# bmds-lab/Crackling

Hardware: AMD Instinct MI355X
Metric: guides/sec (whole node) + achieved HBM GB/s, 20bp/<=4mm ISSL scan (higher is better)
Workload: dtype u32

## Files before the change

crackling_amd/csrc/issl_bin.hip:

```cpp
#include <hip/hip_runtime.h>

#include <algorithm>
#include <type_traits>

#include "issl_kernels.hpp"

namespace issl {


__global__ __launch_bounds__(256) void k_pack_scan_stream(ImageView v, uint32_t *__restrict__ scan_out,
                                                          uint64_t *__restrict__ esig_out,
                                                          uint8_t *__restrict__ occ8_out,
                                                          uint32_t *__restrict__ error_flag, uint32_t *__restrict__ seen,
                                                          uint32_t tile_begin, uint32_t tile_end)
{
    for (uint32_t t = tile_begin + blockIdx.x; t < tile_end; t += gridDim.x) {
        uint32_t lo = 0, hi = v.n_buckets;
        while (hi - lo > 1) {
            const uint32_t mid = (lo + hi) >> 1;
            if (v.tile_first[mid] <= t) lo = mid; else hi = mid;
        }
        const uint32_t b = lo;
        const uint32_t slice = b >> v.slice_width;
        const uint64_t start = v.bucket_start[b];
// ... 463 lines not shown
                                                   ScanItem *__restrict__ fitems, uint32_t item_guides, uint32_t tail_shapes,
                                                   FineItemLds<THREADS> &l)
{
    const uint32_t w = threadIdx.x;
    const FineSum base = fbase[b];
    const uint64_t blen = v.bucket_start[b + 1] - v.bucket_start[b];
    const uint32_t tile_first_b = v.tile_first[b];
    uint32_t c = 0, c1 = 0, s0 = 0, s1 = 0;
    if (w < 256u) {
        c = fcount[static_cast<uint64_t>(b) * 256u + w];
        c1 = c - fcount0[static_cast<uint64_t>(b) * 256u + w];
        const uint32_t *ss = v.sub_start + static_cast<uint64_t>(b) * 257u;
        s0 = ss[w];
        s1 = ss[w + 1];
    }
    uint64_t cost = 0, slots = 0, items = 0;
    GroupUnits gu{};
    if (c) {
        gu = group_units(s0, s1, tail_shapes);
        const uint32_t kk = (c + item_guides - 1u) / item_guides;
        slots = (c + kGuideGroup - 1u) / kGuideGroup * kGuideGroup;
        items = static_cast<uint64_t>(gu.units) * kk;
        for (uint32_t done = 0; done < c; done += item_guides) cost += group_cost(gu, c - done < item_guides ? c - done : item_guides);
    }
    const uint64_t cost_at = base.cost + block_exclusive_scan(cost, l.scan, nullptr);
    const uint32_t slot_at = base.slots + static_cast<uint32_t>(block_exclusive_scan(slots, l.scan, nullptr));
    const uint32_t item_at = static_cast<uint32_t>(block_exclusive_scan(items, l.scan, nullptr));
    if (w < 256u) {
        l.item0_of[w] = item_at;
        if (w == 255u) l.item0_of[256] = item_at + static_cast<uint32_t>(items);
        FineGroup g;
        g.cost0 = cost_at; g.chunk_cost = group_cost(gu, item_guides);
        g.s0 = s0; g.s1 = s1; g.n_full = gu.n_full; g.units = gu.units;
        g.shape = gu.shape; g.c = c; g.slot = slot_at; g.slot0 = slot_at + c1;
        l.group[w] = g;
    }
    __syncthreads();
    const uint32_t total = l.item0_of[256];
    for (uint32_t i0 = 0; i0 < total; i0 += THREADS) {
        const uint32_t i = i0 + w;
        if (i < total) {
            uint32_t lo = 0, hi = 256;
            while (hi - lo > 1u) {
                const uint32_t mid = (lo + hi) >> 1;
                if (l.item0_of[mid] <= i) lo = mid; else hi = mid;
            }
            const uint32_t gw = lo;
            const FineGroup g = l.group[gw];
            const uint32_t s0a = g.s0 & ~31u;
            const uint32_t j = i - l.item0_of[gw];
            const uint32_t chunk = j / g.units, t = j - chunk * g.units;
            const uint32_t done = chunk * item_guides;
            const uint32_t len = (g.c - done < item_guides) ? g.c - done : item_guides;
            const bool full = t < g.n_full;
            const uint32_t shape = full ? 32u : g.shape, cap = 64u * shape;
            const uint32_t wstart = s0a + t * kTileCands;
            const uint64_t after = blen - wstart;
            ScanItem it;
            it.bucket = (b << 8) | gw;
            it.g0 = g.slot + done;
            it.g1 = it.g0 + len;
            it.n_tiles = 1;
            it.cost0 = g.cost0 + static_cast<uint64_t>(chunk) * g.chunk_cost +
                       static_cast<uint64_t>(t) * (static_cast<uint64_t>(len) * kGuideCost + kTileFixedCost);
            it.tile0 = base.items + i;
            it.last_cands = after < cap ? static_cast<uint32_t>(after) : cap;
            it.group_abs = tile_first_b * 64u + (wstart >> 5);
            it.window = (t == 0 ? g.s0 - s0a : 0u) | ((g.s1 - wstart < cap ? g.s1 - wstart : cap) << 16);
            it.shape = shape; it.gmid = g.slot0;
            l.stage[w] = it;
        }
        __syncthreads();
        const uint32_t n_here = total - i0 < THREADS ? total - i0 : THREADS;
        const uint4 *src4 = reinterpret_cast<const uint4 *>(l.stage);
        uint4 *dst4 = reinterpret_cast<uint4 *>(fitems + base.items + i0);
        for (uint32_t q = w; q < n_here * 3u; q += THREADS) dst4[q] = src4[q];
        __syncthreads();
    }
}

template <uint32_t WAYS, uint32_t THREADS>
__device__ __forceinline__ void fine_scatter_guides(const ImageView &v, uint32_t b, const uint32_t *__restrict__ gstart,
                                                    const uint32_t *__restrict__ gfill, const uint32_t *__restrict__ gword,
                                                    const uint32_t *__restrict__ gidx, const uint64_t *__restrict__ gsig,
                                                    const uint32_t *__restrict__ fcount, const uint32_t *__restrict__ fcount0,
                                                    const FineSum *__restrict__ fbase, uint32_t *__restrict__ fword,
                                                    FineMeta *__restrict__ fmeta, FineGuideLds<THREADS> &l)
{
    constexpr uint32_t ways = WAYS;
    const uint32_t w = threadIdx.x, slice = b >> v.slice_width;
    const uint32_t g0 = gstart[b], n = gfill[b];
    const uint32_t base_slots = fbase[b].slots;
    uint32_t c = 0, c1 = 0;
    if (w < 256u) {
        c = fcount[static_cast<uint64_t>(b) * 256u + w];
        c1 = c - fcount0[static_cast<uint64_t>(b) * 256u + w];
    }
    uint32_t i = w, guide = 0, word = 0;
    uint64_t sig = 0;
    if (i < n) { guide = gidx[g0 + i]; word = gword[g0 + i]; sig = gsig[g0 + i]; }
    const uint32_t slots = (c + kGuideGroup - 1u) / kGuideGroup * kGuideGroup;
    const uint32_t slot_at = base_slots + static_cast<uint32_t>(block_exclusive_scan(slots, l.scan, nullptr));
    if (w < 256u) {
        l.slot_of[w] = slot_at;
        l.slot0_of[w] = slot_at + c1;
        l.cursor[w] = 0;
        l.cursor0[w] = 0;
        l.has_cands[w] = c ? 1u : 0u;
        for (uint32_t k2 = c; k2 < slots; ++k2) { fmeta[slot_at + k2] = FineMeta{kNoGuide, 0u, 0ull}; fword[slot_at + k2] = kPadGuideWord; }
    }
    __syncthreads();
    while (i < n) {
        const uint32_t gj = succ_byte(sig, slice, v.slice_width);
        const uint32_t word12 = fine_word(word, slice, v.slice_width);
#pragma unroll
        for (uint32_t way = 0; way < ways; ++way) {
            const uint32_t ww = fine_way(gj, way);
            if (!l.has_cands[ww]) continue;
            const uint32_t slot = way ? l.slot_of[ww] + atomicAdd(&l.cursor[ww], 1u) : l.slot0_of[ww] + atomicAdd(&l.cursor0[ww], 1u);
            fword[slot] = word12 | (fine_class(way) << 24);
            fmeta[slot] = FineMeta{guide, (b << 8) | ww, sig};
        }
        i += THREADS;
        if (i < n) { guide = gidx[g0 + i]; word = gword[g0 + i]; sig = gsig[g0 + i]; }
    }
}

template <uint32_t WAYS, uint32_t THREADS>
__global__ __launch_bounds__(THREADS) void k_fine_scatter(ImageView v, const uint32_t *__restrict__ gstart,
                                                          const uint32_t *__restrict__ gfill, const uint32_t *__restrict__ gword,
                                                          const uint32_t *__restrict__ gidx, const uint64_t *__restrict__ gsig,
                                                          const uint32_t *__restrict__ fcount, const uint32_t *__restrict__ fcount0,
                                                          const FineSum *__restrict__ fbase, const PlanInfo *__restrict__ plan,
                                                          uint32_t *__restrict__ fword, FineMeta *__restrict__ fmeta,
                                                          ScanItem *__restrict__ fitems, uint32_t item_guides, uint32_t tail_shapes)
{
    short_kernel_priority();
    if (!plan->fine) return;
    __shared__ union { FineItemLds<THREADS> items; FineGuideLds<THREADS> guides; } lds;
    const uint32_t nb = v.n_buckets;
    if (blockIdx.x < nb) fine_scatter_items(v, blockIdx.x, fcount, fcount0, fbase, fitems, item_guides, tail_shapes, lds.items);
    else fine_scatter_guides<WAYS, THREADS>(v, blockIdx.x - nb, gstart, gfill, gword, gidx, gsig, fcount, fcount0, fbase, fword, fmeta, lds.guides);
}

__global__ __launch_bounds__(256) void k_fine_ranges(const PlanInfo *__restrict__ plan, const ScanItem *__restrict__ fitems,
                                                     RangeStart *__restrict__ starts)
{
    short_kernel_priority();
    if (!plan->fine) return;
    const uint32_t n_ranges = plan->n_ranges;
    const uint32_t r = blockIdx.x * 4u + (threadIdx.x >> 6);
    if (r <= n_ranges && n_ranges != 0) {
        const RangeStart st = range_start_of<true>(fitems, plan->n_items, plan->total_cost, n_ranges, r);
        if ((threadIdx.x & 63u) == 0u) starts[r] = st;
    }
}

constexpr uint32_t kSmallPairs = 512;

__device__ inline uint64_t block512_exclusive_scan(uint64_t v, uint64_t *lds , uint64_t *total)
{
    const uint32_t lane = threadIdx.x & 63u, wave = threadIdx.x >> 6;
    const uint64_t incl = wave_inclusive_scan_u64(v);
    if (lane == 63) lds[wave] = incl;
    __syncthreads();
    uint64_t before = 0, all = 0;
    for (uint32_t w = 0; w < kSmallPairs / 64u; ++w) {
        const uint64_t x = lds[w];
        if (w < wave) before += x;
        all += x;
    }
    if (total) *total = all;
    __syncthreads();
    return before + incl - v;
}

template <uint32_t WAYS>
__global__ __launch_bounds__(kSmallPairs) void k_bin_small(ImageView v, Workspace ws, const uint64_t *__restrict__ guides, uint32_t n,
                                                           uint32_t prune_mode, uint32_t tail_shapes, uint32_t scan_blocks,
                                                           uint32_t sorted_layout)
{
    short_kernel_priority();
    __shared__ uint64_t lds[kSmallPairs / 64u];
    const uint32_t t = threadIdx.x, my_way = blockIdx.x;
    for (uint32_t k = my_way * kSmallPairs + t; k <= n; k += WAYS * kSmallPairs) ws.gcount[k] = 0;
    for (uint32_t k = my_way * kSmallPairs + t; k <= ws.cap_chunks; k += WAYS * kSmallPairs) ws.raw_used[k] = 0;
    if (t == 0 && my_way == 0) {
        ws.scan_span[2u * ws.span_slot] = ~0ull;
        ws.scan_span[2u * ws.span_slot + 1u] = 0ull;
    }
    const uint32_t pairs = n * v.n_slices;
    const uint32_t low = (1u << v.slice_width) - 1u;
    const bool mine = t < pairs;
    const uint32_t g = mine ? t / v.n_slices : 0u, sl = mine ? t - g * v.n_slices : 0u;
    uint64_t sig = 0, blen = 0, units = 0, cost = 0, cand = 0, ref = 0, valid = 0;
    uint64_t cost_before = 0;
    uint32_t units_before = 0, valid_before = 0;
    uint32_t b = 0, gj = 0, tf = 0, my_s0 = 0, my_s1 = 0;
    if (mine) {
        sig = guides[g];
        b = (sl << v.slice_width) + (static_cast<uint32_t>(sig >> (v.slice_width * sl)) & low);
        gj = succ_byte(sig, sl, v.slice_width);
        const uint32_t *ss = v.sub_start + static_cast<uint64_t>(b) * 257u;
        uint32_t s0[WAYS], s1[WAYS];
#pragma unroll
        for (uint32_t way = 0; way < WAYS; ++way) {
            const uint32_t ww = fine_way(gj, way);
            s0[way] = ss[ww];
            s1[way] = ss[ww + 1];
        }
        blen = v.bucket_start[b + 1] - v.bucket_start[b];
        tf = v.tile_first[b];
        ref = blen;
#pragma unroll
        for (uint32_t way = 0; way < WAYS; ++way) {
            if (way == my_way) { my_s0 = s0[way]; my_s1 = s1[way]; units_before = static_cast<uint32_t>(units); cost_before = cost; valid_before = static_cast<uint32_t>(valid); }
            if (s1[way] > s0[way]) {
                const GroupUnits gu = group_units(s0[way], s1[way], tail_shapes);
                units += gu.units;
                cost += group_cost(gu, 1u);
                cand += s1[way] - s0[way];
                ++valid;
            }
        }
    }
    uint64_t t_units, t_cost, t_cand, t_ref, t_valid;
    uint32_t item_at = static_cast<uint32_t>(block512_exclusive_scan(units, lds, &t_units)) + units_before;
    uint64_t cost_at = block512_exclusive_scan(cost, lds, &t_cost) + cost_before;
    (void)block512_exclusive_scan(cand, lds, &t_cand);
    (void)block512_exclusive_scan(ref, lds, &t_ref);
    const uint32_t slot_at = (static_cast<uint32_t>(block512_exclusive_scan(valid, lds, &t_valid)) + valid_before) * kGuideGroup;
    const uint64_t t_slots = t_valid * kGuideGroup;
    const bool overflow = t_units > ws.cap_fitems || t_slots > ws.cap_fslots;
    if (mine && !overflow && my_s1 > my_s0) {
        const uint32_t way = my_way, s0 = my_s0, s1 = my_s1;
        const uint32_t word12 = fine_word(image_word(sig, sl, v.slice_width, sorted_layout != 0u), sl, v.slice_width);
        const uint32_t ww = fine_way(gj, way);
        const uint32_t c1 = way ? 1u : 0u;
        uint4 *fw = reinterpret_cast<uint4 *>(ws.fword + slot_at);
        fw[0] = make_uint4(word12 | (fine_class(way) << 24), kPadGuideWord, kPadGuideWord, kPadGuideWord);
        fw[1] = make_uint4(kPadGuideWord, kPadGuideWord, kPadGuideWord, kPadGuideWord);
        ws.fmeta[slot_at] = FineMeta{g, (b << 8) | ww, sig};
#pragma unroll
        for (uint32_t k2 = 1; k2 < kGuideGroup; ++k2) ws.fmeta[slot_at + k2] = FineMeta{kNoGuide, 0u, 0ull};
        const GroupUnits gu = group_units(s0, s1, tail_shapes);
        for (uint32_t u = 0; u < gu.units; ++u) {
            const bool full = u < gu.n_full;
            const uint32_t shape = full ? 32u : gu.shape, cap = 64u * shape;
            const uint32_t wstart = gu.s0a + u * kTileCands;
            const uint64_t after = blen - wstart;
            ScanItem it;
            it.bucket = (b << 8) | ww;
            it.g0 = slot_at;
            it.g1 = slot_at + 1u;
            it.n_tiles = 1;
            it.cost0 = cost_at;
            it.tile0 = item_at;
            it.last_cands = after < cap ? static_cast<uint32_t>(after) : cap;
            it.group_abs = tf * 64u + (wstart >> 5);
            it.window = (u == 0 ? s0 - gu.s0a : 0u) | ((s1 - wstart < cap ? s1 - wstart : cap) << 16);
            it.shape = shape; it.gmid = slot_at + c1;
            ws.fitems[item_at++] = it;
            cost_at += static_cast<uint64_t>(shape >> 3) + kTileFixedCost;
        }
    }
    if (t == 0 && my_way == 0) {
        const uint32_t n_items = overflow ? 0u : static_cast<uint32_t>(t_units);
        ScanItem end;
        end.bucket = 0; end.g0 = 0; end.g1 = 0; end.n_tiles = 0; end.cost0 = overflow ? 0ull : t_cost;
        end.tile0 = n_items; end.last_cands = 0; end.group_abs = 0; end.window = 0; end.shape = 32; end.gmid = 0;
        ws.fitems[n_items] = end;
        PlanInfo pl{};
        pl.n_items = n_items;
        pl.error = 0;
        pl.n_ranges = n_items == 0 ? 0u : ranges_for(t_units, scan_blocks);
        pl.fine = prune_mode;
        pl.total_cost = overflow ? 0ull : t_cost;
        pl.candidates = overflow ? 0ull : t_cand;
        pl.reference_candidates = t_ref;
        pl.tiles = n_items;
        pl.fine_slots = overflow ? 0u : static_cast<uint32_t>(t_slots);
        *ws.plan = pl;
        Counters c{};
        c.raw_chunks = (pl.n_ranges ? pl.n_ranges : 1u) * 16u;
        *ws.counters = c;
        if (overflow) {
            atomicMax(&ws.sticky[3], static_cast<uint32_t>(t_units < 0xFFFFFFFFull ? t_units : 0xFFFFFFFFull));
            atomicOr(&ws.sticky[0], 2u);
        }
    }
}

static bool small_bin_ok(const ImageView &v, const Workspace &ws, const Tuning &tn, uint32_t n, uint32_t prune_mode)
{
    if (!tn.small_bin || (prune_mode != 1u && prune_mode != 2u) || !ws.fitems || !v.sub_start) return false;
    if (n == 0 || static_cast<uint64_t>(n) * v.n_slices > kSmallPairs) return false;
    const uint64_t buckets_per_slice = 1ull << v.slice_width;
    return tn.prune == 1 || v.n_sites / buckets_per_slice >= 16ull * kTileCands;
}

uint32_t prune_mode_for(const ImageView &v, const Tuning &tn, uint32_t n_guides, int max_dist)
{
    const bool geometry = v.n_slices * v.slice_width == 40u && (v.slice_width == 8 || v.slice_width == 4 || v.slice_width == 2);
    if ((!v.srec && !v.sid) || tn.prune == 0 || max_dist < 0 || max_dist > 5 || !geometry) return 0;
    if (n_guides > prune_max_guides(max_dist == 5 ? 3u : 2u, v.n_slices)) return 0;
    return max_dist <= 2 ? 1u : max_dist <= 4 ? 2u : 3u;
}

void launch_bin_guides(const ImageView &v, const Workspace &ws, const Tuning &tn, const uint64_t *d_guides, uint32_t n,
                       uint32_t prune_mode, void *stream_)
{
    hipStream_t stream = static_cast<hipStream_t>(stream_);
    const uint32_t nb = v.n_buckets;
    if (small_bin_ok(v, ws, tn, n, prune_mode)) {
        const uint32_t sorted = (v.srec || v.sid) ? 1u : 0u;
        if (fine_ways_of(prune_mode) == 1u)
            hipLaunchKernelGGL(k_bin_small<1u>, dim3(1), dim3(kSmallPairs), 0, stream, v, ws, d_guides, n, prune_mode,
                               static_cast<uint32_t>(tn.tail_shapes), tn.scan_blocks, sorted);
        else
            hipLaunchKernelGGL(k_bin_small<kFineWays>, dim3(kFineWays), dim3(kSmallPairs), 0, stream, v, ws, d_guides, n, prune_mode,
                               static_cast<uint32_t>(tn.tail_shapes), tn.scan_blocks, sorted);
        hipLaunchKernelGGL(k_fine_ranges, dim3((tn.scan_blocks + 1u + 3u) / 4u), dim3(256), 0, stream, ws.plan, ws.fitems, ws.range_start);
        return;
    }
    const uint32_t n_slots = static_cast<uint32_t>(
        std::min<size_t>(ws.cap_gslots, static_cast<size_t>(n) * v.n_slices + static_cast<size_t>(kGuideGroup) * nb));
    const uint32_t blocks = (n + 255u) / 256u;
    const uint32_t reset_blocks = std::min<uint32_t>(1024u, (std::max(n_slots, nb) + 255u) / 256u);
    hipLaunchKernelGGL(k_guide_hist, dim3(std::max(blocks, reset_blocks)), dim3(256), 0, stream, ws, d_guides, n,
                       v.slice_width, v.n_slices, nb, n_slots, tn.scan_blocks * 16u);
    hipLaunchKernelGGL(k_plan, dim3(1), dim3(256), 0, stream, v, ws.ng, ws.gfill, ws.gstart, ws.items,
                       static_cast<uint32_t>(ws.cap_items), ws.plan, tn.item_guides, tn.scan_blocks, ws.counters);
    const uint32_t range_blocks = (tn.scan_blocks + 1u + 255u) / 256u;
    hipLaunchKernelGGL(k_guide_scatter, dim3(blocks + range_blocks), dim3(256), 0, stream, d_guides, n, v.slice_width,
                       v.n_slices, (v.srec || v.sid) ? 1u : 0u, nb, ws.gstart, ws.gfill, ws.gword, ws.gidx, ws.gbucket, ws.gsig, blocks, ws.plan, ws.items,
                       ws.range_start);
    if (prune_mode) {
        const uint32_t ways = fine_ways_of(prune_mode);
        const uint32_t tail_shapes = prune_mode == 3 ? 0u : static_cast<uint32_t>(tn.tail_shapes);
        auto launch_fine = [&](auto ways_tag) {
            constexpr uint32_t W = decltype(ways_tag)::value;
            hipLaunchKernelGGL(k_fine_count<W>, dim3(nb), dim3(256), 0, stream, v, ws.gsig, ws.gstart, ws.gfill, ws.fcount,
                               ws.fcount0, ws.fsum, tn.item_guides, tail_shapes);
            hipLaunchKernelGGL(k_fine_plan, dim3(1), dim3(256), 0, stream, ws.fsum, nb, ws.fitems,
                               static_cast<uint32_t>(ws.cap_fitems), static_cast<uint32_t>(ws.cap_fslots), ws.plan, tn.scan_blocks,
                               prune_mode, tn.prune == 1 ? 1u : 0u, ws.sticky, ws.counters);
            if (static_cast<uint64_t>(n) * v.n_slices > 256ull * nb)
                hipLaunchKernelGGL((k_fine_scatter<W, 512u>), dim3(2u * nb), dim3(512), 0, stream, v, ws.gstart, ws.gfill, ws.gword, ws.gidx, ws.gsig,
                                   ws.fcount, ws.fcount0, ws.fsum, ws.plan, ws.fword, ws.fmeta, ws.fitems, tn.item_guides, tail_shapes);
            else
                hipLaunchKernelGGL((k_fine_scatter<W, 256u>), dim3(2u * nb), dim3(256), 0, stream, v, ws.gstart, ws.gfill, ws.gword, ws.gidx, ws.gsig,
                                   ws.fcount, ws.fcount0, ws.fsum, ws.plan, ws.fword, ws.fmeta, ws.fitems, tn.item_guides, tail_shapes);
        };
        if (ways == 1u) launch_fine(std::integral_constant<uint32_t, 1u>{});
        else if (ways == kFineWays) launch_fine(std::integral_constant<uint32_t, kFineWays>{});
        else launch_fine(std::integral_constant<uint32_t, kFineWays2>{});
        hipLaunchKernelGGL(k_fine_ranges, dim3((tn.scan_blocks + 1u + 3u) / 4u), dim3(256), 0, stream, ws.plan, ws.fitems, ws.range_start);
    }
}

}
```

crackling_amd/csrc/issl_device.hpp:

```cpp
#pragma once
#include <cstddef>
#include <cstdint>
#include <string>

#include "issl_host.hpp"

namespace issl {

constexpr uint64_t kImageMagic = 0x314C535349444D41ull;
constexpr uint32_t kImageVersion = 9;
constexpr uint32_t kTileCands = 2048;
constexpr uint32_t kHeaderBytes = 4096;

struct ImageHeader {
    uint64_t magic;
    uint32_t version;
    uint32_t kind;
    uint64_t n_sites, seq_len, n_lines, slice_width, n_slices, n_scores_file;
    uint64_t n_buckets;
    uint64_t n_scores_unique;
    uint64_t n_tiles;
    uint64_t tile_cands;
    uint64_t total_bytes;
    uint64_t off_bucket_start, off_tile_first, off_score_mask, off_score_val, off_sites, off_entries,
// ... 124 lines not shown
constexpr uint32_t kScanMaxBlocks = 8192u;
constexpr uint32_t kScanWaves = kScanMaxBlocks * 16u;
constexpr uint32_t kMaxRanges = kScanMaxBlocks;
constexpr uint32_t kStampsScanWords = 4u * kScanWaves, kStampsPerReplay = 16u * 4096u;
constexpr uint32_t kStampsMid = kStampsScanWords, kStampsBig256 = kStampsMid + kStampsPerReplay, kStampsBig1024 = kStampsBig256 + kStampsPerReplay;
constexpr uint32_t kStampsWords = kStampsBig1024 + kStampsPerReplay;
constexpr uint32_t kSpanRing = 64;
constexpr uint32_t kChunkRecs = 128;
constexpr uint64_t kDeadKey = ~0ull;
constexpr uint32_t kKeySliceShift = 32, kKeyGuideShift = 37, kKeySliceMask = 31, kMaxSlices = 20;

struct ScanItem {
    uint32_t bucket;
    uint32_t g0, g1;
    uint32_t n_tiles;
    uint64_t cost0;
    uint32_t tile0;
    uint32_t last_cands;
    uint32_t group_abs;
    uint32_t window;
    uint32_t shape;
    uint32_t gmid;
};
static_assert(sizeof(ScanItem) == 48, "scan items are fetched with scalar loads");

struct RangeStart {
    uint32_t item;
    uint32_t tile;
    uint32_t goff;
    uint32_t pad;
};

struct PlanInfo {
    uint32_t n_items;
    uint32_t error;
    uint32_t n_ranges;
    uint32_t fine;
    uint64_t total_cost;
    uint64_t candidates;
    uint64_t reference_candidates;
    uint64_t tiles;
    uint32_t fine_slots;
    uint32_t pad;
};

struct Counters {
    uint32_t next_range;
    uint32_t n_big;
    uint32_t n_big2;
    uint32_t n_big3;
    uint32_t raw_chunks;
    uint32_t raw_overflow;
    uint32_t overflowed;
    uint32_t replay_next[3];
};

struct FineSum {
    uint64_t cost, cand;
    uint32_t slots, items, units;
    uint32_t places;
};

constexpr uint32_t kSlotHits = 512;
constexpr uint32_t kSlotHitsWide = 2048;
struct alignas(32) SlotRec {
    double mit, cfd;
    uint64_t key, pad;
};
#if defined(__HIPCC__)
__host__ __device__
#endif
inline uint64_t slot_pad(uint32_t occ, uint32_t dist) { return static_cast<uint64_t>(occ) | (static_cast<uint64_t>(dist) << 32); }
constexpr uint32_t kFineWays = 13;
constexpr uint32_t kFineWays2 = 67;
constexpr uint32_t kFetchPairs = 8;
constexpr uint32_t kPruneMaxGuides = 1u << 20;
constexpr uint32_t kPruneMaxGuides2 = 1u << 18;
inline uint32_t prune_max_guides(uint32_t prune_mode, uint32_t n_slices)
{
    const uint32_t m = prune_mode == 3 ? kPruneMaxGuides2 : kPruneMaxGuides;
    return n_slices > 10 ? m >> 2 : n_slices > 5 ? m >> 1 : m;
}

struct alignas(16) FineMeta {
    uint32_t guide;
    uint32_t where;
    uint64_t gsig;
};

struct Workspace {
    uint32_t *ng = nullptr;
    uint32_t *gfill = nullptr;
    uint32_t *gstart = nullptr;
    uint32_t *gword = nullptr;
    uint32_t *gidx = nullptr;
    uint32_t *gbucket = nullptr;
    uint64_t *gsig = nullptr;
    ScanItem *items = nullptr;
    uint32_t *fword = nullptr;
    FineMeta *fmeta = nullptr;
    ScanItem *fitems = nullptr;
    uint32_t *fcount = nullptr;
    uint32_t *fcount0 = nullptr;
    FineSum *fsum = nullptr;
    size_t cap_fslots = 0, cap_fitems = 0;
    uint32_t fine_ways = 0;
    PlanInfo *plan = nullptr;
    RangeStart *range_start = nullptr;
    uint64_t *raw = nullptr;
    uint32_t *raw_used = nullptr;
    size_t cap_chunks = 0;
    Counters *counters = nullptr;
    unsigned long long *scan_span = nullptr;
    uint32_t span_slot = 0;
    uint64_t *scan_count = nullptr;
    unsigned long long *stamps = nullptr;
    uint32_t *sticky = nullptr;
    uint64_t *sorted = nullptr;
    uint32_t *gcount = nullptr;
    uint32_t *goff = nullptr;
    uint32_t *gcur_big = nullptr;
    uint32_t *gcur_big2 = nullptr;
    double *terms = nullptr;
    double *pay = nullptr;
    uint32_t *rank = nullptr;
    SlotRec *slots = nullptr;
    uint32_t slot_hits = 0;
    uint32_t slot_width = kSlotHits;
    uint32_t lean_tail = 0;
    size_t cap_slot_guides = 0;
    uint32_t *blocksum = nullptr;
    uint64_t *d_guides = nullptr;
    void *h_stage = nullptr;
    size_t h_stage_bytes = 0;
    double *d_mit = nullptr, *d_cfd = nullptr;
    uint32_t *d_kept = nullptr;
    issl_hit *d_hitrec = nullptr;
    size_t cap_hitrec = 0;
    size_t cap_guides = 0;
    size_t cap_hits = 0;
    size_t cap_items = 0;
    size_t cap_gslots = 0;
    uint32_t n_buckets = 0;
};

struct ScoreParams {
    int max_dist;
    int method;
    double maximum_sum;
};

void launch_pack_scan_stream(const ImageView &v, uint32_t *scan_out, uint64_t *esig_out, uint8_t *occ8_out,
                             uint32_t *error_flag, uint32_t *seen, void *stream);
void launch_pack_scan_range(const ImageView &v, uint32_t *scan_out, uint64_t *esig_out, uint8_t *occ8_out,
                            uint32_t *error_flag, uint32_t *seen, uint32_t tile_begin, uint32_t tile_end, void *stream);
inline uint32_t fine_ways_of(uint32_t prune_mode) { return prune_mode == 1 ? 1u : prune_mode == 3 ? kFineWays2 : kFineWays; }
uint32_t prune_mode_for(const ImageView &v, const Tuning &tn, uint32_t n_guides, int max_dist);
void launch_bin_guides(const ImageView &v, const Workspace &ws, const Tuning &tn, const uint64_t *d_guides, uint32_t n,
                       uint32_t prune_mode, void *stream);
void launch_scan(const ImageView &v, const Workspace &ws, const Tuning &tn, const uint64_t *d_guides, uint32_t n,
                 int max_dist, uint32_t prune_mode, void *stream);
void launch_verify(const ImageView &v, const Workspace &ws, const uint64_t *d_guides, uint32_t n, const ScoreParams &p, void *stream);
void launch_group_hits(const Workspace &ws, uint32_t n, void *stream);
void launch_replay(const ImageView &v, const Workspace &ws, const uint64_t *d_guides, uint32_t n,
                   const ScoreParams &p, double *d_mit, double *d_cfd, uint32_t *d_kept, issl_hit *d_hitrec,
                   void *stream);
void launch_profile(const ImageView &v, const Workspace &ws, const uint64_t *d_guides, uint32_t n, issl_profile *d_out,
                    void *stream);
void launch_report_offsets(const Workspace &ws, uint32_t n, uint64_t base, uint64_t *d_offsets, void *stream);
void launch_report_emit(const ImageView &v, const Workspace &ws, const uint64_t *d_guides, uint32_t n_records,
                        uint32_t guide_base, issl_offtarget *d_out, void *stream);

}
```

crackling_amd/csrc/issl_pipeline.cpp:

```cpp
#include <algorithm>
#include <cstdio>
#include <cstring>
#include <vector>

#include "issl_index.hpp"

namespace issl {

int supported_geometry(const Geometry &g)
{
    if (g.seq_len == 20 && (g.slice_width == 8 || g.slice_width == 4 || g.slice_width == 2) && g.n_slices * g.slice_width == 40) return ISSL_OK;
    set_error("unsupported index geometry: the gfx950 scan kernels implement 20 bp sequences in slices of 8, 4 or 2 bits "
              "(got seq_len=" + std::to_string(g.seq_len) + " slice_width=" +
              std::to_string(g.slice_width) + " slices=" + std::to_string(g.n_slices) + ")");
    return ISSL_E_UNSUPPORTED;
}

int select_device(int device)
{
    int count = 0;
    hipError_t e = hipGetDeviceCount(&count);
    if (e != hipSuccess || count <= 0) {
        set_error("no HIP device available: the ISSL scorer has no CPU fallback");
        return ISSL_E_DEVICE;
    }
    if (device < 0 || device >= count) {
        set_error("device " + std::to_string(device) + " out of range (" + std::to_string(count) + " visible)");
        return ISSL_E_ARG;
    }
    HIP_TRY(hipSetDevice(device));
    return ISSL_OK;
}

static void free_workspace(Workspace &w)
{
    void *ptrs[] = {w.ng, w.gfill, w.gstart, w.gword, w.gidx, w.gbucket, w.gsig, w.items, w.plan, w.range_start, w.counters, w.scan_count, w.scan_span, w.sticky, w.stamps, w.gcur_big, w.gcur_big2, w.terms, w.sorted, w.gcount,
                    w.goff, w.blocksum, w.d_guides, w.d_mit, w.d_cfd, w.d_kept, w.d_hitrec, w.pay, w.rank, w.fword, w.fmeta,
                    w.fitems, w.fcount, w.fcount0, w.fsum, w.slots};
    for (void *p : ptrs)
        if (p) (void)hipFree(p);
    if (w.raw) (void)hipFree(w.raw);
    if (w.raw_used) (void)hipFree(w.raw_used);
    if (w.h_stage) (void)hipHostFree(w.h_stage);
    w = Workspace{};
}

void release_lanes(issl_index *ix)
{
    for (Lane *lp : {&ix->lane, &ix->lane2}) {
        Lane &lane = *lp;
        if (lane.ready) {
            (void)hipStreamSynchronize(lane.stream);
            (void)hipStreamSynchronize(lane.tail_stream);
            for (auto &e : lane.ev) (void)hipEventDestroy(e);
            (void)hipEventDestroy(lane.done);
            (void)hipStreamDestroy(lane.stream);
            (void)hipStreamDestroy(lane.tail_stream);
            lane.ready = false;
        }
        free_workspace(lane.ws);
        lane.lean = false;
        lane.last_n = 0;
        lane.pending = 0;
    }
    ix->last_lane = nullptr;
    if (ix->have_events) {
        for (auto &e : ix->ring) (void)hipEventDestroy(e);
        ix->have_events = false;
    }
    ix->n_pending = 0;
    ix->n_ring = 0;
    ix->proven_guides = 0;
    ix->proven_chunks = 0;
    ix->proven_dist = -1;
    ix->prev_scan_end = nullptr;
    ix->prev_batch_end = nullptr;
}

static bool ensure_stage(Workspace &w, size_t bytes)
{
    if (w.h_stage_bytes >= bytes) return true;
    if (w.h_stage) (void)hipHostFree(w.h_stage);
    w.h_stage = nullptr;
    w.h_stage_bytes = 0;
    const size_t want = bytes + bytes / 4;
    if (hipHostMalloc(&w.h_stage, want, hipHostMallocDefault) != hipSuccess) { (void)hipGetLastError(); w.h_stage = nullptr; return false; }
    w.h_stage_bytes = want;
    return true;
}

template <typename T> static int dev_alloc(T *&p, size_t count)
{
    if (p) {
        (void)hipFree(p);
        p = nullptr;
    }
    HIP_TRY(hipMalloc(reinterpret_cast<void **>(&p), std::max<size_t>(count, 1) * sizeof(T)));
    return ISSL_OK;
}

static int ensure_hit_capacity(Workspace &w, size_t want)
{
    if (want <= w.cap_hits) return ISSL_OK;
    int rc;
    if ((rc = dev_alloc(w.sorted, want))) return rc;
    if ((rc = dev_alloc(w.terms, 2 * want))) return rc;
    if ((rc = dev_alloc(w.pay, 2 * want))) return rc;
    if ((rc = dev_alloc(w.rank, want))) return rc;
    w.cap_hits = want;
    return ISSL_OK;
}

int ensure_raw_capacity(Workspace &w, size_t chunks)
{
    if (chunks <= w.cap_chunks) return ISSL_OK;
    int rc = dev_alloc(w.raw, (chunks + 1) * kChunkRecs);
    if (rc) return rc;
    if ((rc = dev_alloc(w.raw_used, chunks + 1))) return rc;
    w.cap_chunks = chunks;
    return ISSL_OK;
}

int ensure_workspace(issl_index *ix, size_t n, Lane &lane, uint32_t fine_ways)
{
    Workspace &w = lane.ws;
    const Tuning &tn = ix->tuning;
    const size_t nb = ix->hdr.n_buckets;
    int rc;
    if (w.n_buckets != nb) {
        if ((rc = dev_alloc(w.ng, nb))) return rc;
        if ((rc = dev_alloc(w.gfill, nb))) return rc;
        HIP_TRY(hipMemset(w.ng, 0, 4 * nb));
        HIP_TRY(hipMemset(w.gfill, 0, 4 * nb));
        if ((rc = dev_alloc(w.gstart, nb + 1))) return rc;
        if ((rc = dev_alloc(w.counters, 1))) return rc;
        if ((rc = dev_alloc(w.plan, 1))) return rc;
        if ((rc = dev_alloc(w.range_start, kMaxRanges + 2))) return rc;
        if ((rc = dev_alloc(w.scan_count, kScanMaxBlocks))) return rc;
        if ((rc = dev_alloc(w.scan_span, 2 * kSpanRing))) return rc;
        HIP_TRY(hipMemset(w.scan_span, 0, 16 * kSpanRing));
        HIP_TRY(hipMemset(w.scan_count, 0, 8 * kScanMaxBlocks));
        w.n_buckets = static_cast<uint32_t>(nb);
    }
    bool grew = false;
    const bool force_wide = tn.hit_slots == 2 && w.slot_width != kSlotHitsWide &&
                            std::max<size_t>(std::max<size_t>(n, w.cap_guides), 1024) * kSlotHitsWide * sizeof(SlotRec) <= kSlotBytesMax;
    if (force_wide) w.slot_width = kSlotHitsWide;
    if (n > w.cap_guides || (force_wide && w.slots)) {
        grew = true;
        const size_t cap = std::max<size_t>(std::max<size_t>(n, w.cap_guides), 1024);
        const size_t slots = cap * ix->hdr.n_slices + kGuideGroup * nb;
        const size_t items = nb + cap * ix->hdr.n_slices / 8 + 2;
        if ((rc = dev_alloc(w.gword, slots))) return rc;
        if ((rc = dev_alloc(w.gidx, slots))) return rc;
        if ((rc = dev_alloc(w.gbucket, slots))) return rc;
        if ((rc = dev_alloc(w.gsig, slots))) return rc;
        if ((rc = dev_alloc(w.items, items + 1))) return rc;
        if ((rc = dev_alloc(w.gcount, cap + 1))) return rc;
        if ((rc = dev_alloc(w.goff, cap + 1))) return rc;
        if ((rc = dev_alloc(w.gcur_big, cap + 1))) return rc;
        if ((rc = dev_alloc(w.gcur_big2, cap + 1))) return rc;
        if ((rc = dev_alloc(w.blocksum, (cap + 1) / 2048 + 2))) return rc;
        if ((rc = dev_alloc(w.d_guides, cap))) return rc;
        if ((rc = dev_alloc(w.d_mit, cap))) return rc;
        if ((rc = dev_alloc(w.d_cfd, cap))) return rc;
        if ((rc = dev_alloc(w.d_kept, cap))) return rc;
        if (w.slots) { (void)hipFree(w.slots); w.slots = nullptr; }
        w.cap_slot_guides = 0;
        if (cap * w.slot_width * sizeof(SlotRec) > kSlotBytesMax) w.slot_width = kSlotHits;
        if (cap * w.slot_width * sizeof(SlotRec) <= kSlotBytesMax) {
            if (hipMalloc(reinterpret_cast<void **>(&w.slots), cap * w.slot_width * sizeof(SlotRec)) == hipSuccess) w.cap_slot_guides = cap;
            else { (void)hipGetLastError(); w.slots = nullptr; }
        }
        w.cap_guides = cap;
        w.cap_gslots = slots;
        w.cap_items = items;
    }
    if (ix->hdr.off_sub_start && (grew || fine_ways > w.fine_ways)) {
        const size_t cap = w.cap_guides;
        const uint32_t ways = std::max(fine_ways, w.fine_ways);
        const size_t m = std::min<size_t>(cap, prune_max_guides(ways > kFineWays ? 3u : 2u, ix->hdr.n_slices));
        const size_t places = m * ix->hdr.n_slices * ways;
        const size_t groups = std::min<size_t>(nb * 256, places);
        const size_t fslots = places + kGuideGroup * groups;
        const size_t tiles_per_group = static_cast<size_t>(ix->hdr.n_sites * ix->hdr.n_slices / (static_cast<uint64_t>(nb) * 256ull * kTileCands)) + 4;
        const size_t fitems = std::max<size_t>(tn.fine_items ? tn.fine_items : tiles_per_group * (groups + places / 64) + 2, w.cap_fitems);
        if ((rc = dev_alloc(w.fword, fslots + 64))) return rc;
        if ((rc = dev_alloc(w.fmeta, fslots))) return rc;
        if ((rc = dev_alloc(w.fitems, fitems + 1))) return rc;
        if ((rc = dev_alloc(w.fcount, nb * 256))) return rc;
        if ((rc = dev_alloc(w.fcount0, nb * 256))) return rc;
        if ((rc = dev_alloc(w.fsum, nb))) return rc;
        w.cap_fslots = fslots;
        w.cap_fitems = fitems;
        w.fine_ways = ways;
    }

    if (w.cap_chunks == 0) {
        const size_t want = tn.raw_chunks ? tn.raw_chunks : std::max<size_t>(size_t(scan_waves(tn)) * 6, n);
        if ((rc = ensure_raw_capacity(w, want))) return rc;
    }
    if (!ix->have_events) {
        for (auto &e : ix->ring) HIP_TRY(hipEventCreate(&e));
        ix->have_events = true;
    }
    if (!lane.ready) {
        for (auto &e : lane.ev) HIP_TRY(hipEventCreate(&e));
        HIP_TRY(hipEventCreate(&lane.done));
        int prio_low = 0, prio_high = 0;
        HIP_TRY(hipDeviceGetStreamPriorityRange(&prio_low, &prio_high));
        HIP_TRY(hipStreamCreateWithPriority(&lane.stream, hipStreamNonBlocking, prio_low));
        HIP_TRY(hipStreamCreateWithPriority(&lane.tail_stream, hipStreamNonBlocking, prio_high));
        lane.ready = true;
    }
    if (!w.stamps && !tn.stamps_path.empty()) {
        if ((rc = dev_alloc(w.stamps, kStampsWords))) return rc;
        HIP_TRY(hipMemset(w.stamps, 0, 8ull * kStampsWords));
    }
    if (!w.sticky) {
        if ((rc = dev_alloc(w.sticky, 4))) return rc;
        HIP_TRY(hipMemset(w.sticky, 0, 16));
    }
    return ISSL_OK;
}

static int enqueue_batch(issl_index *ix, Lane &lane, hipStream_t stream, const uint64_t *d_guides, size_t n, int max_dist,
                         double threshold, int method, double *d_mit, double *d_cfd, bool dump, bool staged,
                         int lanes_mode = 1, issl_profile *d_profile = nullptr)
{
    const bool pipelined = lanes_mode == 2, bin_ahead = lanes_mode == 3;
    if (!ix->d_image) {
        set_error("index has no device image: call issl_index_upload first");
        return ISSL_E_STATE;
    }
    const size_t max_batch = std::min<size_t>(kMaxBatch, ((size_t(1) << 27) - kGuideGroup * ix->hdr.n_buckets) / std::max<uint64_t>(ix->hdr.n_slices, 1));
    if (n > max_batch) {
        set_error("at most " + std::to_string(max_batch) + " guides per device batch on this index (issl_score splits larger batches itself)");
        return ISSL_E_ARG;
    }
    HIP_TRY(hipSetDevice(ix->device));
    if (n == 0) return ISSL_OK;
    const uint32_t prune_mode = prune_mode_for(ix->view, ix->tuning, static_cast<uint32_t>(n), max_dist);
    int rc = ensure_workspace(ix, n, lane, fine_ways_of(prune_mode ? prune_mode : 2u));
    if (rc) return rc;
    Workspace &ws = lane.ws;
    const Tuning &tn = ix->tuning;
    rc = ensure_hit_capacity(ws, ws.cap_chunks * (kChunkRecs - 1));
    if (rc) return rc;
    if (dump && ws.cap_hitrec < ws.cap_hits) {
        rc = dev_alloc(ws.d_hitrec, ws.cap_hits);
        if (rc) return rc;
        ws.cap_hitrec = ws.cap_hits;
    }
    ws.slot_hits = (!dump && tn.hit_slots && ws.cap_slot_guides >= n) ? ws.slot_width : 0u;
    ws.lean_tail = (lane.lean && ws.slot_hits >= kSlotHits && tn.lean_tail) ? 1u : 0u;
    ScoreParams p;
    p.max_dist = max_dist;
    p.method = method;
    p.maximum_sum = (10000.0 - threshold * 100) / threshold;
    const uint32_t n32 = static_cast<uint32_t>(n);
    const bool scan_pair = staged || pipelined || tn.scan_events == 1 || (tn.scan_events == 2 && ix->n_ring == 0);
    const uint32_t slot = ix->n_ring % kRing;
    lane.staged = staged;
    if (pipelined && lane.pending) HIP_TRY(hipStreamWaitEvent(stream, lane.done, 0));
    if (staged) HIP_TRY(hipEventRecord(lane.ev[0], stream));
    ws.span_slot = lane.pending % kSpanRing;
    launch_bin_guides(ix->view, ws, tn, d_guides, n32, prune_mode, stream);
    if (staged) HIP_TRY(hipEventRecord(lane.ev[1], stream));
    if (pipelined && ix->prev_scan_end) HIP_TRY(hipStreamWaitEvent(stream, ix->prev_scan_end, 0));
    if (bin_ahead && ix->prev_batch_end) HIP_TRY(hipStreamWaitEvent(stream, ix->prev_batch_end, 0));
    if (scan_pair) HIP_TRY(hipEventRecord(ix->ring[2 * slot], stream));
// ... 484 lines not shown
```

crackling_amd/csrc/issl_verify.hip:

```cpp
#include <hip/hip_runtime.h>

#include <algorithm>

#include "issl_kernels.hpp"

namespace issl {

__global__ __launch_bounds__(kChunkRecs, 8) void k_verify(ImageView v, Workspace ws, const uint64_t *__restrict__ guides,
                                                       ScoreParams p)
{
    short_kernel_priority();
    const int max_dist = p.max_dist;
    const bool calc_mit = p.method == ISSL_METHOD_MIT || p.method == ISSL_METHOD_AND || p.method == ISSL_METHOD_OR ||
                          p.method == ISSL_METHOD_AVG;
    const bool calc_cfd = p.method == ISSL_METHOD_CFD || p.method == ISSL_METHOD_AND || p.method == ISSL_METHOD_OR ||
                          p.method == ISSL_METHOD_AVG;
    const uint32_t prune_mode = ws.plan->fine;
    uint32_t n_chunks = ws.counters->raw_chunks;
    if (blockIdx.x == 0 && threadIdx.x == 0) {
        if (ws.counters->raw_overflow) atomicOr(&ws.sticky[0], 1u);
        atomicMax(&ws.sticky[1], n_chunks);
        if (ws.plan->error) atomicOr(&ws.sticky[2], ws.plan->error);
    }
    if (n_chunks > ws.cap_chunks) n_chunks = static_cast<uint32_t>(ws.cap_chunks);
    const uint64_t low = (1ull << v.slice_width) - 1ull;
    for (uint32_t chunk = blockIdx.x; chunk < n_chunks; chunk += gridDim.x) {
        uint64_t *recs = ws.raw + static_cast<uint64_t>(chunk) * kChunkRecs;
        const uint32_t t = threadIdx.x + 1u;
        const uint64_t rec_any = recs[t < kChunkRecs ? t : 0u];
        const uint32_t used = ws.raw_used[chunk];
        const bool in_use = t < used && t < kChunkRecs;
        const uint64_t rec = in_use ? rec_any : 0ull;
        uint64_t key = kDeadKey;
        double mit_term = 0.0, cfd_term = 0.0;
        uint64_t hit_gsig = 0, hit_ot = 0;
        uint32_t hit_occ = 0;
        const uint32_t offset = static_cast<uint32_t>(rec) & (kTileCands - 1u);
        const uint32_t tile = static_cast<uint32_t>(rec >> 11) & 0x3FFFFFFu;
        const uint32_t gslot = static_cast<uint32_t>(rec >> 37);
        const bool by_id = v.srec || v.sid;
        StreamRec sr_early{};
        if (in_use && v.srec) sr_early = v.srec[static_cast<uint64_t>(tile) * kTileCands + offset];
        else if (in_use && v.sid) sr_early.id = v.sid[static_cast<uint64_t>(tile) * kTileCands + offset];
        uint32_t guide = kNoGuide, where = 0;
        uint64_t gsig = 0;
        if (in_use) {
            if (prune_mode) { const FineMeta m = ws.fmeta[gslot]; guide = m.guide; where = m.where; gsig = m.gsig; }
            else { guide = ws.gidx[gslot]; where = ws.gbucket[gslot]; }
        }
        if (guide != kNoGuide) {
            const uint32_t bucket = prune_mode ? where >> 8 : where;
            const uint32_t slice = bucket >> v.slice_width;
            uint64_t start = 0, pos = 0;
            bool mine = true;
            if (!by_id) {
                start = v.bucket_start[bucket];
                pos = static_cast<uint64_t>(tile - v.tile_first[bucket]) * kTileCands + offset;
                mine = pos < v.bucket_start[bucket + 1] - start;
            }
            if (mine) {
                if (!prune_mode) gsig = guides[guide];
                StreamRec sr = sr_early;
                if (v.sid) sr.sig = v.sites[sr.id];
                const uint64_t ot = by_id    ? sr.sig & kSigMask
                                    : v.esig ? v.esig[start + pos]
                                    : v.occ8 ? candidate_signature(v, bucket, tile, offset)
                                             : v.sites[v.entries[start + pos] & 0xFFFFFFFFull];
                if (__builtin_popcountll(mismatch_mask(gsig, ot)) <= max_dist) {
                    const uint64_t x = gsig ^ ot;
                    if (!prune_mode) {
                        bool earlier = false;
                        for (uint32_t j = 0; j < slice; ++j)
                            if (((x >> (v.slice_width * j)) & low) == 0) earlier = true;
                        if (!earlier) {
                            const uint64_t lp = by_id ? sr.id : pos;
                            key = (static_cast<uint64_t>(guide) << kKeyGuideShift) | (static_cast<uint64_t>(slice) << kKeySliceShift) | lp;
                        }
                    } else {
                        const uint32_t tol = prune_mode - 1u;
                        const uint64_t mm = mismatch_mask(gsig, ot);
                        uint32_t first = slice, reporter = slice;
                        for (uint32_t j = slice; j-- > 0;) {
                            if (((x >> (v.slice_width * j)) & low) != 0) continue;
                            first = j;
                            if (static_cast<uint32_t>(__builtin_popcount(succ_byte(mm, j, v.slice_width))) <= tol) reporter = j;
                        }
                        if (reporter == slice)
                            key = (static_cast<uint64_t>(guide) << kKeyGuideShift) | (static_cast<uint64_t>(first) << kKeySliceShift) | sr.id;
                    }
                    if (key != kDeadKey) {
                        uint32_t occ;
                        if (by_id) {
                            occ = static_cast<uint32_t>(sr.sig >> 40);
                            if (occ == kOccSaturated) occ = v.site_occ[sr.id];
                        } else if (v.occ8) {
                            occ = v.occ8[start + pos];
                            if (occ == 255u) occ = static_cast<uint32_t>(v.entries[start + pos] >> 32);
                        } else {
                            occ = static_cast<uint32_t>(v.entries[start + pos] >> 32);
                        }
                        hit_gsig = gsig; hit_ot = ot; hit_occ = occ;
                    }
                }
            }
        }
        const bool live = key != kDeadKey;
        const uint32_t lane = threadIdx.x & 63u;
        const uint32_t prev_guide = static_cast<uint32_t>(__shfl_up(static_cast<int>(live ? guide : kNoGuide), 1, 64));
        const bool continues = live && lane != 0u && prev_guide == guide;
        const uint64_t starts = __ballot(!continues);
        uint32_t rank = 0;
        if (starts == ~0ull) {
            if (live) rank = atomicAdd(&ws.gcount[guide], 1u);
        } else {
            const uint64_t upto = (lane == 63u ? 0ull : (~0ull << (lane + 1u)));
            const uint32_t head = 63u - static_cast<uint32_t>(__builtin_clzll(starts & ~upto));
            const uint64_t later = starts & upto;
            const uint32_t next = later ? static_cast<uint32_t>(__builtin_ctzll(later)) : 64u;
            uint32_t base = 0;
            if (live && !continues) base = atomicAdd(&ws.gcount[guide], next - lane);
            rank = static_cast<uint32_t>(__shfl(static_cast<int>(base), static_cast<int>(head), 64)) + (lane - head);
        }
        if (live && rank == kReplayLds) atomicAdd(&ws.counters->overflowed, 1u);
        if (live && rank < ws.slot_hits) {
            int dist;
            score_terms(v, hit_gsig, hit_ot, hit_occ, calc_mit, calc_cfd, mit_term, cfd_term, dist);
            const uint64_t at = static_cast<uint64_t>(guide) * ws.slot_hits + rank;
            SlotRec r;
            r.mit = mit_term; r.cfd = cfd_term; r.key = key;
            r.pad = slot_pad(hit_occ, static_cast<uint32_t>(dist));
            ws.slots[at] = r;
            key = kDeadKey;
        } else if (live) {
            const uint64_t slot = static_cast<uint64_t>(chunk) * (kChunkRecs - 1u) + (t - 1u);
// ... 21 lines not shown
```

Before: 44.32 million.

## Replace 16-byte fine slot metadata with a 4-byte index into guide arrays

The fine scatter path no longer writes a 16-byte FineMeta record (guide, bucket/way, signature) per fine slot. It writes a 32-bit index into the existing gidx/gbucket/gsig arrays, and the small-pair path now fills those arrays for its own guides. Verify gets the guide, bucket and signature through one extra indirection. This cuts scatter write traffic and fine-slot memory, at the cost of a dependent second load in verify. The way bits that were packed into `where` are dropped.

```diff
diff --git a/crackling_amd/csrc/issl_bin.hip b/crackling_amd/csrc/issl_bin.hip
--- a/crackling_amd/csrc/issl_bin.hip
+++ b/crackling_amd/csrc/issl_bin.hip
@@ -569,10 +569,10 @@
 template <uint32_t WAYS, uint32_t THREADS>
 __device__ __forceinline__ void fine_scatter_guides(const ImageView &v, uint32_t b, const uint32_t *__restrict__ gstart,
                                                     const uint32_t *__restrict__ gfill, const uint32_t *__restrict__ gword,
-                                                    const uint32_t *__restrict__ gidx, const uint64_t *__restrict__ gsig,
+                                                    const uint64_t *__restrict__ gsig,
                                                     const uint32_t *__restrict__ fcount, const uint32_t *__restrict__ fcount0,
                                                     const FineSum *__restrict__ fbase, uint32_t *__restrict__ fword,
-                                                    FineMeta *__restrict__ fmeta, FineGuideLds<THREADS> &l)
+                                                    uint32_t *__restrict__ fpair, FineGuideLds<THREADS> &l)
 {
     constexpr uint32_t ways = WAYS;
     const uint32_t w = threadIdx.x, slice = b >> v.slice_width;
@@ -583,9 +583,9 @@
         c = fcount[static_cast<uint64_t>(b) * 256u + w];
         c1 = c - fcount0[static_cast<uint64_t>(b) * 256u + w];
     }
-    uint32_t i = w, guide = 0, word = 0;
+    uint32_t i = w, word = 0;
     uint64_t sig = 0;
-    if (i < n) { guide = gidx[g0 + i]; word = gword[g0 + i]; sig = gsig[g0 + i]; }
+    if (i < n) { word = gword[g0 + i]; sig = gsig[g0 + i]; }
     const uint32_t slots = (c + kGuideGroup - 1u) / kGuideGroup * kGuideGroup;
     const uint32_t slot_at = base_slots + static_cast<uint32_t>(block_exclusive_scan(slots, l.scan, nullptr));
     if (w < 256u) {
@@ -594,7 +594,7 @@
         l.cursor[w] = 0;
         l.cursor0[w] = 0;
         l.has_cands[w] = c ? 1u : 0u;
-        for (uint32_t k2 = c; k2 < slots; ++k2) { fmeta[slot_at + k2] = FineMeta{kNoGuide, 0u, 0ull}; fword[slot_at + k2] = kPadGuideWord; }
+        for (uint32_t k2 = c; k2 < slots; ++k2) { fpair[slot_at + k2] = kNoGuide; fword[slot_at + k2] = kPadGuideWord; }
     }
     __syncthreads();
     while (i < n) {
@@ -606,20 +606,20 @@
             if (!l.has_cands[ww]) continue;
             const uint32_t slot = way ? l.slot_of[ww] + atomicAdd(&l.cursor[ww], 1u) : l.slot0_of[ww] + atomicAdd(&l.cursor0[ww], 1u);
             fword[slot] = word12 | (fine_class(way) << 24);
-            fmeta[slot] = FineMeta{guide, (b << 8) | ww, sig};
+            fpair[slot] = g0 + i;
         }
         i += THREADS;
-        if (i < n) { guide = gidx[g0 + i]; word = gword[g0 + i]; sig = gsig[g0 + i]; }
+        if (i < n) { word = gword[g0 + i]; sig = gsig[g0 + i]; }
     }
 }
 
 template <uint32_t WAYS, uint32_t THREADS>
 __global__ __launch_bounds__(THREADS) void k_fine_scatter(ImageView v, const uint32_t *__restrict__ gstart,
                                                           const uint32_t *__restrict__ gfill, const uint32_t *__restrict__ gword,
-                                                          const uint32_t *__restrict__ gidx, const uint64_t *__restrict__ gsig,
+                                                          const uint64_t *__restrict__ gsig,
                                                           const uint32_t *__restrict__ fcount, const uint32_t *__restrict__ fcount0,
                                                           const FineSum *__restrict__ fbase, const PlanInfo *__restrict__ plan,
-                                                          uint32_t *__restrict__ fword, FineMeta *__restrict__ fmeta,
+                                                          uint32_t *__restrict__ fword, uint32_t *__restrict__ fpair,
                                                           ScanItem *__restrict__ fitems, uint32_t item_guides, uint32_t tail_shapes)
 {
     short_kernel_priority();
@@ -627,7 +627,7 @@
     __shared__ union { FineItemLds<THREADS> items; FineGuideLds<THREADS> guides; } lds;
     const uint32_t nb = v.n_buckets;
     if (blockIdx.x < nb) fine_scatter_items(v, blockIdx.x, fcount, fcount0, fbase, fitems, item_guides, tail_shapes, lds.items);
-    else fine_scatter_guides<WAYS, THREADS>(v, blockIdx.x - nb, gstart, gfill, gword, gidx, gsig, fcount, fcount0, fbase, fword, fmeta, lds.guides);
+    else fine_scatter_guides<WAYS, THREADS>(v, blockIdx.x - nb, gstart, gfill, gword, gsig, fcount, fcount0, fbase, fword, fpair, lds.guides);
 }
 
 __global__ __launch_bounds__(256) void k_fine_ranges(const PlanInfo *__restrict__ plan, const ScanItem *__restrict__ fitems,
@@ -719,6 +719,7 @@
     const uint32_t slot_at = (static_cast<uint32_t>(block512_exclusive_scan(valid, lds, &t_valid)) + valid_before) * kGuideGroup;
     const uint64_t t_slots = t_valid * kGuideGroup;
     const bool overflow = t_units > ws.cap_fitems || t_slots > ws.cap_fslots;
+    if (mine && my_way == 0) { ws.gidx[t] = g; ws.gbucket[t] = b; ws.gsig[t] = sig; }
     if (mine && !overflow && my_s1 > my_s0) {
         const uint32_t way = my_way, s0 = my_s0, s1 = my_s1;
         const uint32_t word12 = fine_word(image_word(sig, sl, v.slice_width, sorted_layout != 0u), sl, v.slice_width);
@@ -727,9 +728,9 @@
         uint4 *fw = reinterpret_cast<uint4 *>(ws.fword + slot_at);
         fw[0] = make_uint4(word12 | (fine_class(way) << 24), kPadGuideWord, kPadGuideWord, kPadGuideWord);
         fw[1] = make_uint4(kPadGuideWord, kPadGuideWord, kPadGuideWord, kPadGuideWord);
-        ws.fmeta[slot_at] = FineMeta{g, (b << 8) | ww, sig};
-#pragma unroll
-        for (uint32_t k2 = 1; k2 < kGuideGroup; ++k2) ws.fmeta[slot_at + k2] = FineMeta{kNoGuide, 0u, 0ull};
+        uint4 *fp = reinterpret_cast<uint4 *>(ws.fpair + slot_at);
+        fp[0] = make_uint4(t, kNoGuide, kNoGuide, kNoGuide);
+        fp[1] = make_uint4(kNoGuide, kNoGuide, kNoGuide, kNoGuide);
         const GroupUnits gu = group_units(s0, s1, tail_shapes);
         for (uint32_t u = 0; u < gu.units; ++u) {
             const bool full = u < gu.n_full;
@@ -833,11 +834,11 @@
                                static_cast<uint32_t>(ws.cap_fitems), static_cast<uint32_t>(ws.cap_fslots), ws.plan, tn.scan_blocks,
                                prune_mode, tn.prune == 1 ? 1u : 0u, ws.sticky, ws.counters);
             if (static_cast<uint64_t>(n) * v.n_slices > 256ull * nb)
-                hipLaunchKernelGGL((k_fine_scatter<W, 512u>), dim3(2u * nb), dim3(512), 0, stream, v, ws.gstart, ws.gfill, ws.gword, ws.gidx, ws.gsig,
-                                   ws.fcount, ws.fcount0, ws.fsum, ws.plan, ws.fword, ws.fmeta, ws.fitems, tn.item_guides, tail_shapes);
+                hipLaunchKernelGGL((k_fine_scatter<W, 512u>), dim3(2u * nb), dim3(512), 0, stream, v, ws.gstart, ws.gfill, ws.gword, ws.gsig,
+                                   ws.fcount, ws.fcount0, ws.fsum, ws.plan, ws.fword, ws.fpair, ws.fitems, tn.item_guides, tail_shapes);
             else
-                hipLaunchKernelGGL((k_fine_scatter<W, 256u>), dim3(2u * nb), dim3(256), 0, stream, v, ws.gstart, ws.gfill, ws.gword, ws.gidx, ws.gsig,
-                                   ws.fcount, ws.fcount0, ws.fsum, ws.plan, ws.fword, ws.fmeta, ws.fitems, tn.item_guides, tail_shapes);
+                hipLaunchKernelGGL((k_fine_scatter<W, 256u>), dim3(2u * nb), dim3(256), 0, stream, v, ws.gstart, ws.gfill, ws.gword, ws.gsig,
+                                   ws.fcount, ws.fcount0, ws.fsum, ws.plan, ws.fword, ws.fpair, ws.fitems, tn.item_guides, tail_shapes);
         };
         if (ways == 1u) launch_fine(std::integral_constant<uint32_t, 1u>{});
         else if (ways == kFineWays) launch_fine(std::integral_constant<uint32_t, kFineWays>{});
diff --git a/crackling_amd/csrc/issl_device.hpp b/crackling_amd/csrc/issl_device.hpp
--- a/crackling_amd/csrc/issl_device.hpp
+++ b/crackling_amd/csrc/issl_device.hpp
@@ -230,11 +230,6 @@
     return n_slices > 10 ? m >> 2 : n_slices > 5 ? m >> 1 : m;
 }
 
-struct alignas(16) FineMeta {
-    uint32_t guide;
-    uint32_t where;
-    uint64_t gsig;
-};
 
 struct Workspace {
     uint32_t *ng = nullptr;
@@ -246,7 +241,7 @@
     uint64_t *gsig = nullptr;
     ScanItem *items = nullptr;
     uint32_t *fword = nullptr;
-    FineMeta *fmeta = nullptr;
+    uint32_t *fpair = nullptr;
     ScanItem *fitems = nullptr;
     uint32_t *fcount = nullptr;
     uint32_t *fcount0 = nullptr;
diff --git a/crackling_amd/csrc/issl_pipeline.cpp b/crackling_amd/csrc/issl_pipeline.cpp
--- a/crackling_amd/csrc/issl_pipeline.cpp
+++ b/crackling_amd/csrc/issl_pipeline.cpp
@@ -35,7 +35,7 @@
 static void free_workspace(Workspace &w)
 {
     void *ptrs[] = {w.ng, w.gfill, w.gstart, w.gword, w.gidx, w.gbucket, w.gsig, w.items, w.plan, w.range_start, w.counters, w.scan_count, w.scan_span, w.sticky, w.stamps, w.gcur_big, w.gcur_big2, w.terms, w.sorted, w.gcount,
-                    w.goff, w.blocksum, w.d_guides, w.d_mit, w.d_cfd, w.d_kept, w.d_hitrec, w.pay, w.rank, w.fword, w.fmeta,
+                    w.goff, w.blocksum, w.d_guides, w.d_mit, w.d_cfd, w.d_kept, w.d_hitrec, w.pay, w.rank, w.fword, w.fpair,
                     w.fitems, w.fcount, w.fcount0, w.fsum, w.slots};
     for (void *p : ptrs)
         if (p) (void)hipFree(p);
@@ -186,7 +186,7 @@
         const size_t tiles_per_group = static_cast<size_t>(ix->hdr.n_sites * ix->hdr.n_slices / (static_cast<uint64_t>(nb) * 256ull * kTileCands)) + 4;
         const size_t fitems = std::max<size_t>(tn.fine_items ? tn.fine_items : tiles_per_group * (groups + places / 64) + 2, w.cap_fitems);
         if ((rc = dev_alloc(w.fword, fslots + 64))) return rc;
-        if ((rc = dev_alloc(w.fmeta, fslots))) return rc;
+        if ((rc = dev_alloc(w.fpair, fslots))) return rc;
         if ((rc = dev_alloc(w.fitems, fitems + 1))) return rc;
         if ((rc = dev_alloc(w.fcount, nb * 256))) return rc;
         if ((rc = dev_alloc(w.fcount0, nb * 256))) return rc;
diff --git a/crackling_amd/csrc/issl_verify.hip b/crackling_amd/csrc/issl_verify.hip
--- a/crackling_amd/csrc/issl_verify.hip
+++ b/crackling_amd/csrc/issl_verify.hip
@@ -42,14 +42,16 @@
         StreamRec sr_early{};
         if (in_use && v.srec) sr_early = v.srec[static_cast<uint64_t>(tile) * kTileCands + offset];
         else if (in_use && v.sid) sr_early.id = v.sid[static_cast<uint64_t>(tile) * kTileCands + offset];
-        uint32_t guide = kNoGuide, where = 0;
+        uint32_t pair = kNoGuide;
+        if (in_use) pair = prune_mode ? ws.fpair[gslot] : gslot;
+        uint32_t guide = kNoGuide, bucket = 0;
         uint64_t gsig = 0;
-        if (in_use) {
-            if (prune_mode) { const FineMeta m = ws.fmeta[gslot]; guide = m.guide; where = m.where; gsig = m.gsig; }
-            else { guide = ws.gidx[gslot]; where = ws.gbucket[gslot]; }
+        if (pair != kNoGuide) {
+            guide = ws.gidx[pair];
+            bucket = ws.gbucket[pair];
+            if (prune_mode) gsig = ws.gsig[pair];
         }
         if (guide != kNoGuide) {
-            const uint32_t bucket = prune_mode ? where >> 8 : where;
             const uint32_t slice = bucket >> v.slice_width;
             uint64_t start = 0, pos = 0;
             bool mine = true;
```

Result: no change. 44.15 million (-0.4%).
